# CompVis/stable-diffusion

Measured on AMD Instinct MI355X. Metric: 512x512 images/sec, SD-v1-4 50-step PLMS CFG=7.5, higher is better.
Workload: dtype f16

## Files before the change

include/sdmi.h:

```cpp
#ifndef SDMI_H_
#define SDMI_H_

#include <stdint.h>

#ifdef __cplusplus
extern "C" {
#endif

#define SDMI_ABI_VERSION 17

typedef struct sdmi_unet sdmi_unet;

typedef struct sdmi_unet_cfg {
  int32_t in_channels;
  int32_t out_channels;
  int32_t model_channels;
  int32_t num_res_blocks;
  int32_t n_levels;
  int32_t channel_mult[8];
  int32_t n_attention_resolutions;
  int32_t attention_resolutions[8];
  int32_t num_heads;
  int32_t transformer_depth;
  int32_t context_dim;
// ... 237 lines not shown
                      float* out, int64_t ldo, void* stream);

typedef struct sdmi_igemm_desc {
  const void* a0; const void* a1; const void* a2;
  int32_t c0, c1, c2, lda0, lda1, lda2;
  int32_t B, Hin, Win, Hout, Wout, ksize, stride, up;
  const void* w;
  int32_t N;
  int32_t mode;
  const float* bias; const float* rowvec; int32_t ld_rowvec;
  const float* residual; int32_t ldr;
  float* out_f32; void* out_f16; int32_t ldo;
  void* seg_dst[3]; int32_t seg_kind[3];
  int32_t heads, dh, ntok, ntok_pad, segC;
  int32_t splitk;
  float* splitk_ws; int64_t splitk_ws_floats;
  int32_t tile;
  int32_t dma;
  int32_t asym_pad;
  int32_t gn_n; void* gn_acc[2]; int32_t gn_cpg[2]; int32_t gn_cbase[2];
  int32_t* splitk_cnt; int32_t splitk_cnt_ints;
  int32_t split16;
  const float* f16_scale; float* lnp_out;
  const float* lnf_part; int32_t lnf_npart; float lnf_eps; const float* lnf_cs; const float* lnf_d;
  const float* pgn_gamma; const float* pgn_beta; float pgn_eps; int32_t pgn_silu;
  void* pgn_out; int32_t pgn_keep_f32; int32_t* pgn_applied;
  void* out_lo;
} sdmi_igemm_desc;
int sdmi_k_igemm(const sdmi_igemm_desc* d, void* stream);
int sdmi_k_igemm_tail(const sdmi_igemm_desc* d, const void* t0, const void* t1, const void* t2, int tail_c, int tail_ld, const void* tail_w,
                      int tail_kt, void* stream);
int sdmi_k_tail_split_range(int nkt, int nsplit, int split, int* begin, int* end);
int sdmi_k_igemm_up_phase(const sdmi_igemm_desc* d, void* stream);
int sdmi_k_up_phase_weights(const void* w_packed_f16, void* dst_f16, int N, int Cin, void* stream);
int sdmi_k_ff_tail(const sdmi_igemm_desc* proj_out, const void* ln_f16, const float* lnp, float ln_eps, const float* csd,
                   const void* wgg_f16, const void* wff2_f16, const float* bff2, const float* t, void* stream);
int sdmi_k_st_tail(const sdmi_igemm_desc* proj_out, const void* a_f16, const void* wo_f16, const float* bo, float* t, const float* ln_gamma,
                   float ln_eps, const float* csd, const void* wgg_f16, const void* wff2_f16, const float* bff2, void* stream);
int sdmi_k_gn_conv3(const sdmi_igemm_desc* conv, const float* x0, const float* x1, int c0, int c1, float* gn_ws, int64_t gn_ws_floats,
                    const float* gn_gamma, const float* gn_beta, float gn_eps, void* stream);
int sdmi_k_st_head(const float* x, float* gn_ws, int64_t gn_ws_floats, const float* gn_gamma, const float* gn_beta, float gn_eps,
                   const void* w_in3, const float* b_in, float* t, const float* ln_gamma, float ln_eps, const void* wqkv_f16,
                   const float* lnf_cs, const float* lnf_d, void* q, void* k, void* vt, int B, int ntok, int ntok_pad, int heads, int dh,
                   int C, void* stream);
int sdmi_k_st_mid(const void* a_f16, const void* wo_f16, const float* bo, float* t, const float* ln_gamma, float ln_eps, const void* wq_f16,
                  const float* lnf_cs, const float* lnf_d, void* q, int B, int ntok, int heads, int dh, int C, void* stream);
int sdmi_k_st_mid_ctx(const void* a_f16, const void* wo_f16, const float* bo, float* t, const float* ln_gamma, float ln_eps, const void* wq_f16,
                      const float* lnf_cs, const float* lnf_d, const void* ctx_k, const void* ctx_vt, int nkv, int nkv_pad, float scale, void* ao_out,
                      int B, int ntok, int heads, int dh, int C, void* stream);
int sdmi_k_ln_fold_prep(const void* w_f16, int N, int K, int ldw, const float* gamma, const float* beta, const float* bias,
                        float* cs, float* d, void* stream);
int sdmi_k_attention(const void* q, const void* k, const void* vt, void* out, int BH, int heads, int nq, int nkv,
                     int nkv_pad, int d, float scale, void* stream);
int sdmi_k_attention_split16(const void* q, const void* q_lo, const void* k, const void* k_lo, const void* vt, const void* vt_lo, void* out,
                             void* out_lo, int BH, int heads, int nq, int nkv, int nkv_pad, int d, float scale, void* stream);
int sdmi_k_attention_split16_causal(const void* q, const void* q_lo, const void* k, const void* k_lo, const void* vt, const void* vt_lo,
                                    void* out, void* out_lo, int BH, int heads, int n, int n_pad, int d, float scale, void* stream);
int sdmi_k_attention_causal(const void* q, const void* k, const void* vt, void* out, int BH, int heads, int n, int n_pad,
                            int d, float scale, void* stream);
int sdmi_k_groupnorm(const float* x0, const float* x1, int c0, int c1, int B, int HW, const float* gamma,
                     const float* beta, float eps, int silu, void* out_f16, float* out_f32, void* raw_f16, void* out_lo,
                     void* raw_lo, float* partial_ws, int64_t partial_floats, void* stream);
int64_t sdmi_k_groupnorm_ws_floats(int B, int HW);
int sdmi_k_groupnorm_film(const float* x0, const float* x1, int c0, int c1, int B, int HW, const float* gamma, const float* beta, float eps,
                          int silu, const float* film, int film_ld, void* out_f16, float* out_f32, void* raw_f16, void* out_lo, void* raw_lo,
                          float* partial_ws, int64_t partial_floats, void* stream);
int sdmi_k_layernorm(const float* x, const float* gamma, const float* beta, void* out_f16, int M, int C, float eps,
                     void* stream);
int sdmi_k_cast_f16(const float* x, void* out_f16, void* out_lo, int64_t n, void* stream);
int sdmi_k_split_heads(const float* src, int ld, int col0, void* dst, void* dst_lo, int kind, int B, int ntok, int ntok_pad, int heads, int dh,
                       void* stream);
int sdmi_k_geglu_split(const float* src, int M, int F, void* out, void* out_lo, void* stream);
int sdmi_k_layernorm_split(const float* x, const float* gamma, const float* beta, void* out, void* out_lo, int M, int C, float eps, void* stream);
int sdmi_k_timestep_embedding(const int64_t* t_i64, const float* t_f32, float* out, int B, int dim, void* stream);
int sdmi_k_small_linear(const float* in, int ld_in, const float* w, const float* bias, float* out, int ld_out, int B,
                        int N, int K, int silu_in, void* stream);
int sdmi_k_conv_in(const float* x_nchw, const float* w_oihw, const float* bias, float* out_nhwc, int B, int Cin, int H,
                   int W, int Cout, void* stream);
int sdmi_k_conv_out(const float* h_nhwc, const float* w_ohwi, const float* bias, float* out_nchw, int B, int H, int W,
                    int Cin, int Cout, void* stream);
int sdmi_k_conv_out32(const float* h_nhwc, const float* w_ohwi, const float* bias, float* out_nchw, int B, int H, int W,
                      int Cin, int Cout, void* stream);
int sdmi_k_conv_in64(const float* x_nchw, const float* w_oihw, const float* bias, float* out_nhwc, int B, int Cin, int H, int W,
                     int Cout, void* stream);
int sdmi_k_conv_out128(const float* h_nhwc, const float* w_ohwi, const float* bias, float* out_nchw, int B, int H, int W, int Cin,
                       int Cout, void* stream);
int sdmi_k_pack_conv_weight(const float* w_oihw, void* dst_f16, int O, int I, int KH, int KW, void* stream);
int sdmi_k_pack_conv_weight_src(const float* w_oihw, void* dst_f16, int O, int I, int KH, int KW, int c0, int c1, int c2, void* stream);
int sdmi_k_pack_conv_out(const float* w_oihw, float* dst_ohwi, int O, int I, void* stream);
int sdmi_k_pack_split3(const float* w, void* dst_f16, int N, int K, void* stream);
int sdmi_k_pack_conv_split3(const float* w_oihw, void* dst_f16, int O, int I, int KH, int KW, void* stream);
int sdmi_k_pointwise_nchw(const float* x, const float* w, const float* bias, float* out, int B, int Cin, int Cout, int HW,
                          float in_scale, void* stream);
int sdmi_k_pointwise_nchw128(const float* x, const float* w, const float* bias, float* out, int B, int Cin, int Cout, int HW,
                             float in_scale, void* stream);
int sdmi_k_softmax_rows(const float* S, void* P_f16, int rows, int cols, float scale, void* stream);
int sdmi_k_vq_quantize(const float* z, float z_scale, const float* codebook, float* norms_ws, int n_embed, int D, float* zq, int32_t* idx,
                       int B, int HW, void* stream);
int sdmi_k_resample2(const float* x, float* out_f32, void* out_f16, void* out_lo, int B, int H, int W, int C, int dir, void* stream);
int sdmi_k_patch_unfold(const float* x, const float* c, float* out, int B, int Cx, int Cc, int H, int W, int kh, int kw, int sy, int sx,
                        int l0, int nl, void* stream);
int sdmi_k_patch_fold(const float* o, const float* w, float* out, int B, int C, int H, int W, int kh, int kw, int sy, int sx, int uf, int df,
                      int norm_only, void* stream);
int sdmi_k_spatial_rescale(const float* x, const float* w, const float* bias, float* out, int B, int Cin, int H, int W, int n_stages,
                           int Cout, void* stream);
int sdmi_k_spatial_rescale_labels(const int32_t* labels, const float* w, const float* bias, float* out, int B, int Cin, int H, int W,
// ... 24 lines not shown
```

stable-diffusion_amd/_lib.py:

```python
import ctypes as C
import os

_HERE = os.path.dirname(os.path.abspath(__file__))
LIB_PATH = os.environ.get('SDMI_LIB_PATH') or os.path.join(_HERE, 'libsdmi.so')

c_f32p = C.c_void_p
c_ptr = C.c_void_p


class UNetCfg(C.Structure):
    _fields_ = [('in_channels', C.c_int32), ('out_channels', C.c_int32), ('model_channels', C.c_int32),
                ('num_res_blocks', C.c_int32), ('n_levels', C.c_int32), ('channel_mult', C.c_int32 * 8),
                ('n_attention_resolutions', C.c_int32), ('attention_resolutions', C.c_int32 * 8),
                ('num_heads', C.c_int32), ('transformer_depth', C.c_int32), ('context_dim', C.c_int32)]


class VaeCfg(C.Structure):
    _fields_ = [('ch', C.c_int32), ('out_ch', C.c_int32), ('n_levels', C.c_int32), ('ch_mult', C.c_int32 * 8),
                ('num_res_blocks', C.c_int32), ('in_channels', C.c_int32), ('z_channels', C.c_int32),
                ('embed_dim', C.c_int32)]


class UNetExt(C.Structure):
    _fields_ = [('attention_block', C.c_int32), ('resblock_updown', C.c_int32)]
# ... 152 lines not shown
    'sdmi_k_safety_head': (C.c_int, [c_ptr, c_ptr, c_ptr, c_ptr, c_ptr, c_ptr, c_ptr, c_ptr, C.c_int, C.c_int, C.c_int, C.c_int, c_ptr]),
    'sdmi_fe_ksize': (C.c_int, [C.c_int, C.c_int]),
    'sdmi_fe_coeffs': (C.c_int, [C.c_int, C.c_int, c_ptr, c_ptr]),
    'sdmi_fe_output_size': (C.c_int, [C.c_int, C.c_int, C.c_int, C.POINTER(C.c_int), C.POINTER(C.c_int)]),
    'sdmi_fe_workspace_bytes': (C.c_int64, [C.c_int] * 5),
    'sdmi_k_clip_feature_extract': (C.c_int, [c_ptr] + [C.c_int] * 7 + [c_ptr, c_ptr, C.c_int, c_ptr, c_ptr, C.c_int, C.POINTER(C.c_float),
                                              C.POINTER(C.c_float), c_ptr, C.c_int64, c_ptr, c_ptr, c_ptr]),
    'sdmi_knn_create': (C.c_int, [C.c_int, C.c_int64, C.POINTER(c_ptr)]),
    'sdmi_knn_destroy': (C.c_int, [c_ptr]),
    'sdmi_knn_set_rows': (C.c_int, [c_ptr, C.c_int64, C.c_int64, c_ptr, c_ptr]),
    'sdmi_knn_finalize': (C.c_int, [c_ptr, c_ptr]),
    'sdmi_knn_rows': (C.c_int64, [c_ptr]),
    'sdmi_knn_dim': (C.c_int, [c_ptr]),
    'sdmi_knn_workspace_bytes': (C.c_int64, [c_ptr, C.c_int, C.c_int]),
    'sdmi_knn_search': (C.c_int, [c_ptr, c_ptr, C.c_int, C.c_int, c_ptr, c_ptr, c_ptr, c_ptr, C.c_int64, c_ptr]),
    'sdmi_knn_condition': (C.c_int, [c_ptr, c_ptr, C.c_int, C.c_int, c_ptr, c_ptr, c_ptr, c_ptr, C.c_int64, c_ptr]),
    'sdmi_k_knn_inv_norm': (C.c_int, [c_ptr, C.c_int64, C.c_int, c_ptr, c_ptr]),
    'sdmi_k_knn_scan': (C.c_int, [c_ptr, c_ptr, C.c_int64, C.c_int, c_ptr, C.c_int, C.c_int, C.c_int64, c_ptr, c_ptr, c_ptr]),
    'sdmi_k_knn_merge': (C.c_int, [c_ptr, c_ptr, C.c_int, C.c_int, C.c_int, c_ptr, c_ptr, c_ptr]),
    'sdmi_k_knn_stream_read': (C.c_int, [c_ptr, C.c_int64, c_ptr, c_ptr]),
    'sdmi_k_knn_gather': (C.c_int, [c_ptr, c_ptr, C.c_int64, C.c_int, c_ptr, C.c_int, C.c_int, c_ptr, c_ptr, C.c_int64, c_ptr]),
    'sdmi_has_experiments': (C.c_int, []),
    'sdmi_k_igemm': (C.c_int, [C.POINTER(IGemmDesc), c_ptr]),
    'sdmi_k_igemm_tail': (C.c_int, [C.POINTER(IGemmDesc), c_ptr, c_ptr, c_ptr, C.c_int, C.c_int, c_ptr, C.c_int, c_ptr]),
    'sdmi_k_tail_split_range': (C.c_int, [C.c_int, C.c_int, C.c_int, C.POINTER(C.c_int), C.POINTER(C.c_int)]),
    'sdmi_k_igemm_up_phase': (C.c_int, [C.POINTER(IGemmDesc), c_ptr]),
    'sdmi_k_up_phase_weights': (C.c_int, [c_ptr, c_ptr, C.c_int, C.c_int, c_ptr]),
    'sdmi_tune_lookup': (C.c_int, [C.c_int] * 9 + [C.POINTER(C.c_int), C.POINTER(C.c_int)]),
    'sdmi_unet_skip_fold_plan': (C.c_int, [c_ptr, C.c_int, C.c_int, C.c_int, C.c_int, C.POINTER(C.c_int32), C.c_int]),
    'sdmi_k_ff_tail': (C.c_int, [C.POINTER(IGemmDesc), c_ptr, c_ptr, C.c_float, c_ptr, c_ptr, c_ptr, c_ptr, c_ptr, c_ptr]),
    'sdmi_k_gn_conv3': (C.c_int, [C.POINTER(IGemmDesc), c_ptr, c_ptr, C.c_int, C.c_int, c_ptr, C.c_int64, c_ptr, c_ptr, C.c_float, c_ptr]),
    'sdmi_k_st_mid_ctx': (C.c_int, [c_ptr, c_ptr, c_ptr, c_ptr, c_ptr, C.c_float, c_ptr, c_ptr, c_ptr, c_ptr, c_ptr, C.c_int, C.c_int, C.c_float, c_ptr,
                                    C.c_int, C.c_int, C.c_int, C.c_int, C.c_int, c_ptr]),
    'sdmi_k_st_tail': (C.c_int, [C.POINTER(IGemmDesc), c_ptr, c_ptr, c_ptr, c_ptr, c_ptr, C.c_float, c_ptr, c_ptr, c_ptr, c_ptr, c_ptr]),
    'sdmi_k_st_mid': (C.c_int, [c_ptr, c_ptr, c_ptr, c_ptr, c_ptr, C.c_float, c_ptr, c_ptr, c_ptr, c_ptr, C.c_int, C.c_int, C.c_int, C.c_int,
                                C.c_int, c_ptr]),
    'sdmi_k_st_head': (C.c_int, [c_ptr, c_ptr, C.c_int64, c_ptr, c_ptr, C.c_float, c_ptr, c_ptr, c_ptr, c_ptr, C.c_float, c_ptr, c_ptr, c_ptr,
                                 c_ptr, c_ptr, c_ptr, C.c_int, C.c_int, C.c_int, C.c_int, C.c_int, C.c_int, c_ptr]),
    'sdmi_k_attention_split16': (C.c_int, [c_ptr, c_ptr, c_ptr, c_ptr, c_ptr, c_ptr, c_ptr, c_ptr, C.c_int, C.c_int, C.c_int, C.c_int,
                                           C.c_int, C.c_int, C.c_float, c_ptr]),
    'sdmi_k_attention_split16_causal': (C.c_int, [c_ptr, c_ptr, c_ptr, c_ptr, c_ptr, c_ptr, c_ptr, c_ptr, C.c_int, C.c_int, C.c_int, C.c_int,
                                                  C.c_int, C.c_float, c_ptr]),
    'sdmi_k_attention_causal': (C.c_int, [c_ptr, c_ptr, c_ptr, c_ptr, C.c_int, C.c_int, C.c_int, C.c_int, C.c_int, C.c_float,
                                          c_ptr]),
    'sdmi_k_pointwise_nchw': (C.c_int, [c_ptr, c_ptr, c_ptr, c_ptr, C.c_int, C.c_int, C.c_int, C.c_int, C.c_float, c_ptr]),
    'sdmi_k_pointwise_nchw128': (C.c_int, [c_ptr, c_ptr, c_ptr, c_ptr, C.c_int, C.c_int, C.c_int, C.c_int, C.c_float, c_ptr]),
    'sdmi_k_softmax_rows': (C.c_int, [c_ptr, c_ptr, C.c_int, C.c_int, C.c_float, c_ptr]),
    'sdmi_k_gelu_erf': (C.c_int, [c_ptr, c_ptr, C.c_int64, c_ptr]),
    'sdmi_k_quick_gelu': (C.c_int, [c_ptr, c_ptr, C.c_int64, c_ptr]),
    'sdmi_k_quick_gelu_split': (C.c_int, [c_ptr, c_ptr, c_ptr, C.c_int64, c_ptr]),
    'sdmi_k_gelu_erf_split': (C.c_int, [c_ptr, c_ptr, c_ptr, C.c_int64, c_ptr]),
    'sdmi_k_attention': (C.c_int, [c_ptr, c_ptr, c_ptr, c_ptr, C.c_int, C.c_int, C.c_int, C.c_int, C.c_int, C.c_int,
                                   C.c_float, c_ptr]),
    'sdmi_k_groupnorm': (C.c_int, [c_ptr, c_ptr, C.c_int, C.c_int, C.c_int, C.c_int, c_ptr, c_ptr, C.c_float, C.c_int,
                                   c_ptr, c_ptr, c_ptr, c_ptr, c_ptr, c_ptr, C.c_int64, c_ptr]),
    'sdmi_k_groupnorm_ws_floats': (C.c_int64, [C.c_int, C.c_int]),
    'sdmi_k_groupnorm_film': (C.c_int, [c_ptr, c_ptr, C.c_int, C.c_int, C.c_int, C.c_int, c_ptr, c_ptr, C.c_float, C.c_int, c_ptr, C.c_int,
                                        c_ptr, c_ptr, c_ptr, c_ptr, c_ptr, c_ptr, C.c_int64, c_ptr]),
    'sdmi_k_layernorm': (C.c_int, [c_ptr, c_ptr, c_ptr, c_ptr, C.c_int, C.c_int, C.c_float, c_ptr]),
    'sdmi_k_cast_f16': (C.c_int, [c_ptr, c_ptr, c_ptr, C.c_int64, c_ptr]),
    'sdmi_k_split_heads': (C.c_int, [c_ptr, C.c_int, C.c_int, c_ptr, c_ptr, C.c_int, C.c_int, C.c_int, C.c_int, C.c_int, C.c_int,
                                     c_ptr]),
    'sdmi_k_geglu_split': (C.c_int, [c_ptr, C.c_int, C.c_int, c_ptr, c_ptr, c_ptr]),
    'sdmi_k_layernorm_split': (C.c_int, [c_ptr, c_ptr, c_ptr, c_ptr, c_ptr, C.c_int, C.c_int, C.c_float, c_ptr]),
    'sdmi_k_timestep_embedding': (C.c_int, [c_ptr, c_ptr, c_ptr, C.c_int, C.c_int, c_ptr]),
    'sdmi_k_small_linear': (C.c_int, [c_ptr, C.c_int, c_ptr, c_ptr, c_ptr, C.c_int, C.c_int, C.c_int, C.c_int,
                                      C.c_int, c_ptr]),
    'sdmi_k_conv_in': (C.c_int, [c_ptr, c_ptr, c_ptr, c_ptr, C.c_int, C.c_int, C.c_int, C.c_int, C.c_int, c_ptr]),
    'sdmi_k_conv_out': (C.c_int, [c_ptr, c_ptr, c_ptr, c_ptr, C.c_int, C.c_int, C.c_int, C.c_int, C.c_int, c_ptr]),
    'sdmi_k_pack_conv_weight': (C.c_int, [c_ptr, c_ptr, C.c_int, C.c_int, C.c_int, C.c_int, c_ptr]),
    'sdmi_k_pack_conv_weight_src': (C.c_int, [c_ptr, c_ptr, C.c_int, C.c_int, C.c_int, C.c_int, C.c_int, C.c_int, C.c_int, c_ptr]),
    'sdmi_k_conv_out32': (C.c_int, [c_ptr, c_ptr, c_ptr, c_ptr, C.c_int, C.c_int, C.c_int, C.c_int, C.c_int, c_ptr]),
    'sdmi_k_conv_in64': (C.c_int, [c_ptr, c_ptr, c_ptr, c_ptr, C.c_int, C.c_int, C.c_int, C.c_int, C.c_int, c_ptr]),
    'sdmi_k_conv_out128': (C.c_int, [c_ptr, c_ptr, c_ptr, c_ptr, C.c_int, C.c_int, C.c_int, C.c_int, C.c_int, c_ptr]),
    'sdmi_k_pack_conv_out': (C.c_int, [c_ptr, c_ptr, C.c_int, C.c_int, c_ptr]),
    'sdmi_k_pack_split3': (C.c_int, [c_ptr, c_ptr, C.c_int, C.c_int, c_ptr]),
    'sdmi_k_pack_conv_split3': (C.c_int, [c_ptr, c_ptr, C.c_int, C.c_int, C.c_int, C.c_int, c_ptr]),
    'sdmi_k_pack_geglu': (C.c_int, [c_ptr, c_ptr, c_ptr, c_ptr, C.c_int, C.c_int, c_ptr]),
    'sdmi_k_ln_fold_prep': (C.c_int, [c_ptr, C.c_int, C.c_int, C.c_int, c_ptr, c_ptr, c_ptr, c_ptr, c_ptr, c_ptr]),
    'sdmi_image_to_uint8': (C.c_int, [c_ptr, c_ptr, C.c_int, C.c_int, C.c_int, C.c_int, c_ptr]),
    'sdmi_range_check': (C.c_int, [C.c_int]),
    'sdmi_range_report': (C.c_int, [C.c_char_p, C.c_int]),
    'sdmi_tune_begin': (C.c_int, []),
    'sdmi_tune_round': (C.c_int, [C.c_int]),
    'sdmi_tune_end': (C.c_int, [C.c_char_p, C.POINTER(C.c_int)]),
    'sdmi_tune_dump': (C.c_int, [C.c_char_p, C.c_int]),
    'sdmi_profile_begin': (C.c_int, []),
    'sdmi_profile_end': (C.c_int, [C.c_char_p, C.c_int]),
    'sdmi_k_prefetch_lines': (C.c_int, [c_ptr, C.c_int64, c_ptr]),
    'sdmi_zero_page': (c_ptr, []),
}

_lib = None


class SdmiError(RuntimeError):
    pass


def load():
    global _lib
    if _lib is None:
        if not os.path.exists(LIB_PATH):
            raise SdmiError(f'{LIB_PATH} not found: build it with `python stable-diffusion_amd/build.py` '
                            '(the MI355X path has no fallback implementation)')
        lib = C.CDLL(LIB_PATH)
# ... 27 lines not shown
```

stable-diffusion_amd/build.py:

```python
import concurrent.futures as cf
import hashlib
import os
import subprocess
import sys

HERE = os.path.dirname(os.path.abspath(__file__))
CSRC = os.path.join(HERE, 'csrc')
EXTRA = os.environ.get('SDMI_CXXFLAGS', '').split()
LIB = os.path.join(HERE, os.environ.get('SDMI_LIB_OUT', 'libsdmi.so'))
OBJ = os.path.join(HERE, 'build' if os.path.basename(LIB) == 'libsdmi.so' else 'build_' + os.path.splitext(os.path.basename(LIB))[0])
SOURCES = ['igemm_t1.hip', 'igemm_t0.hip', 'igemm_t2.hip', 'igemm_h1.hip', 'igemm_h0.hip', 'igemm_h2.hip', 'igemm.hip', 'conv3halo.hip', 'gemm_split16.hip', 'rowchain.hip', 'gnconv.hip', 'range.hip', 'attn.hip', 'attn_wide.hip', 'attn_split16.hip', 'attn_wide_split16.hip', 'split_ops.hip', 'norm.hip', 'small.hip', 'sampler.hip', 'dpm.hip', 'inpaint.hip', 'patch.hip', 'vit.hip', 'knn.hip', 'textpool.hip', 'rescale.hip', 'feature_extractor.hip', 'fe_coeffs.cpp', 'weights.cpp', 'unet.cpp', 'vae.cpp', 'clip.cpp', 'bert.cpp', 'api.cpp', 'prof.cpp']
NO_CONTRACT = ('sampler.hip', 'dpm.hip', 'feature_extractor.hip', 'fe_coeffs.cpp')
FLAGS = ['--offload-arch=gfx950', '-O3', '-std=c++17', '-fPIC', '-munsafe-fp-atomics', '-Wall', '-Wno-unused-function',
         '-Wno-unused-variable']


def _hipcc():
    for c in (os.environ.get('HIPCC'), '/opt/rocm/bin/hipcc', 'hipcc'):
        if c and (not os.path.isabs(c) or os.path.exists(c)):
            return c
    raise RuntimeError('hipcc not found')


def _stamp():
    h = hashlib.sha256()
    for root in (CSRC, os.path.join(os.path.dirname(HERE), 'include')):
        for fn in sorted(os.listdir(root)):
            with open(os.path.join(root, fn), 'rb') as f:
                h.update(fn.encode())
                h.update(f.read())
    h.update(' '.join(FLAGS + EXTRA).encode())
    return h.hexdigest()


def is_current():
    stamp_file = os.path.join(OBJ, 'stamp')
    return os.path.exists(LIB) and os.path.exists(stamp_file) and open(stamp_file).read() == _stamp()


def build(force=False, verbose=True):
    os.makedirs(OBJ, exist_ok=True)
    stamp_file = os.path.join(OBJ, 'stamp')
    if not force and is_current():
        return LIB
    hipcc = _hipcc()
    stamp_now = _stamp()

    inc_dirs = (CSRC, os.path.join(os.path.dirname(HERE), 'include'))

    def deps_hash(src):
        import re
        seen, todo, h = set(), [os.path.join(CSRC, src)], hashlib.sha256()
        while todo:
            path = todo.pop()
            if path in seen:
                continue
            seen.add(path)
            with open(path, 'rb') as f:
                data = f.read()
            h.update(os.path.basename(path).encode())
            h.update(data)
            for inc in re.findall(rb'^\s*#\s*include\s*"([^"]+)"', data, re.M):
                for d in (os.path.dirname(path),) + inc_dirs:
                    cand = os.path.join(d, inc.decode())
# ... 37 lines not shown
```

stable-diffusion_amd/csrc/api.cpp:

```cpp
#include <string.h>

#include <new>

#include "prof.h"
#include "split16.h"
#include "unet.h"
#include "vae.h"
#include "clip.h"
#include "knn.h"
#include "rescale.h"
#include "fe_coeffs.h"
#include "feature_extractor.h"
#include "sampler_rows.h"

namespace sdmi {
static thread_local std::string g_err;
void set_error(const std::string& msg) { g_err = msg; }
int fail(const std::string& msg) { g_err = msg; return -1; }
}

struct sdmi_unet { sdmi::UNet impl; };
struct sdmi_vae { sdmi::Vae impl; };
struct sdmi_clip { sdmi::ClipText impl; };
struct sdmi_bert { sdmi::BertText impl; };
// ... 676 lines not shown
  if (launch_groupnorm(g, (hipStream_t)stream)) return -1;
  q.x0 = x0; q.x1 = x1; q.c0 = c0; q.c1 = c1; q.gn_acc = (const long long*)gn_ws; q.gn_gamma = gn_gamma; q.gn_beta = gn_beta; q.gn_eps = gn_eps;
  q.w = (const f16*)conv->w;
  return launch_gn_conv3(q, (hipStream_t)stream);
}
int sdmi_k_st_head(const float* x, float* gn_ws, int64_t gn_ws_floats, const float* gn_gamma, const float* gn_beta, float gn_eps,
                   const void* w_in3, const float* b_in, float* t, const float* ln_gamma, float ln_eps, const void* wqkv_f16,
                   const float* lnf_cs, const float* lnf_d, void* q, void* k, void* vt, int B, int ntok, int ntok_pad, int heads, int dh,
                   int C, void* stream) {
  SDMI_CHECK(x && gn_ws && gn_gamma && gn_beta, "st_head: null argument");
  SDMI_CHECK(gn_ws_floats >= gn_acc_words(B) * 2, "groupnorm workspace too small");
  SDMI_HIP_OK(hipMemsetAsync(gn_ws, 0, gn_acc_words(B) * sizeof(long long), (hipStream_t)stream));
  GroupNormParams g = GroupNormParams();
  g.x0 = x; g.c0 = C; g.B = B; g.HW = ntok; g.gamma = gn_gamma; g.beta = gn_beta; g.eps = gn_eps; g.stats_only = 1; g.acc = (long long*)gn_ws;
  if (launch_groupnorm(g, (hipStream_t)stream)) return -1;
  StHeadParams p = StHeadParams();
  p.x = x; p.gn_acc = (const long long*)gn_ws; p.gn_gamma = gn_gamma; p.gn_beta = gn_beta; p.gn_eps = gn_eps;
  p.w_in = (const f16*)w_in3; p.b_in = b_in; p.t = t; p.ln_gamma = ln_gamma; p.ln_eps = ln_eps; p.wqkv = (const f16*)wqkv_f16;
  p.lnf_cs = lnf_cs; p.lnf_d = lnf_d; p.q = (f16*)q; p.k = (f16*)k; p.vt = (f16*)vt;
  p.M = B * ntok; p.B = B; p.ntok = ntok; p.ntok_pad = ntok_pad; p.heads = heads; p.dh = dh; p.C = C;
  return launch_st_head(p, (hipStream_t)stream);
}
int sdmi_k_st_mid(const void* a_f16, const void* wo_f16, const float* bo, float* t, const float* ln_gamma, float ln_eps, const void* wq_f16,
                  const float* lnf_cs, const float* lnf_d, void* q, int B, int ntok, int heads, int dh, int C, void* stream) {
  StHeadParams p = StHeadParams();
  p.a16 = (const f16*)a_f16; p.w_in = (const f16*)wo_f16; p.b_in = bo; p.t = t; p.ln_gamma = ln_gamma; p.ln_eps = ln_eps;
  p.wqkv = (const f16*)wq_f16; p.lnf_cs = lnf_cs; p.lnf_d = lnf_d; p.q = (f16*)q;
  p.M = B * ntok; p.B = B; p.ntok = ntok; p.ntok_pad = ntok; p.heads = heads; p.dh = dh; p.C = C;
  return launch_st_mid(p, (hipStream_t)stream);
}
int sdmi_k_st_mid_ctx(const void* a_f16, const void* wo_f16, const float* bo, float* t, const float* ln_gamma, float ln_eps, const void* wq_f16,
                      const float* lnf_cs, const float* lnf_d, const void* ctx_k, const void* ctx_vt, int nkv, int nkv_pad, float scale, void* ao_out,
                      int B, int ntok, int heads, int dh, int C, void* stream) {
  StHeadParams p = StHeadParams();
  p.a16 = (const f16*)a_f16; p.w_in = (const f16*)wo_f16; p.b_in = bo; p.t = t; p.ln_gamma = ln_gamma; p.ln_eps = ln_eps;
  p.wqkv = (const f16*)wq_f16; p.lnf_cs = lnf_cs; p.lnf_d = lnf_d;
  p.ctx_k = (const f16*)ctx_k; p.ctx_vt = (const f16*)ctx_vt; p.ctx_nkv = nkv; p.ctx_nkv_pad = nkv_pad; p.ctx_scale = scale; p.ao_out = (f16*)ao_out;
  SDMI_CHECK(ctx_k && ctx_vt && ao_out, "st_mid_ctx: null argument");
  p.M = B * ntok; p.B = B; p.ntok = ntok; p.ntok_pad = ntok; p.heads = heads; p.dh = dh; p.C = C;
  return launch_st_mid(p, (hipStream_t)stream);
}
int sdmi_k_ln_fold_prep(const void* w_f16, int N, int K, int ldw, const float* gamma, const float* beta, const float* bias,
                        float* cs, float* d, void* stream) {
  return launch_ln_fold_prep((const f16*)w_f16, N, K, ldw, gamma, beta, bias, cs, d, (hipStream_t)stream);
}
int sdmi_k_attention(const void* q, const void* k, const void* vt, void* out, int BH, int heads, int nq, int nkv,
                     int nkv_pad, int d, float scale, void* stream) {
  AttnParams a = AttnParams();
  a.q = (const f16*)q; a.k = (const f16*)k; a.vt = (const f16*)vt; a.out = (f16*)out;
  a.BH = BH; a.heads = heads; a.nq = nq; a.nkv = nkv; a.nkv_pad = nkv_pad; a.d = d; a.scale = scale;
  if (const char* e = getenv("SDMI_ATTN_NW")) a.nw = atoi(e);
  return launch_attention(a, (hipStream_t)stream);
}
int sdmi_k_attention_split16(const void* q, const void* q_lo, const void* k, const void* k_lo, const void* vt, const void* vt_lo, void* out,
                             void* out_lo, int BH, int heads, int nq, int nkv, int nkv_pad, int d, float scale, void* stream) {
  AttnSplitParams a = AttnSplitParams();
  a.q = (const f16*)q; a.q_lo = (const f16*)q_lo; a.k = (const f16*)k; a.k_lo = (const f16*)k_lo; a.vt = (const f16*)vt;
  a.vt_lo = (const f16*)vt_lo; a.out = (f16*)out; a.out_lo = (f16*)out_lo;
  a.BH = BH; a.heads = heads; a.nq = nq; a.nkv = nkv; a.nkv_pad = nkv_pad; a.d = d; a.scale = scale;
  return launch_attention_split16(a, (hipStream_t)stream);
}
int64_t sdmi_k_groupnorm_ws_floats(int B, int HW) { (void)HW; return gn_acc_words(B) * 2; }
int sdmi_k_groupnorm(const float* x0, const float* x1, int c0, int c1, int B, int HW, const float* gamma,
                     const float* beta, float eps, int silu, void* out_f16, float* out_f32, void* raw_f16, void* out_lo,
                     void* raw_lo, float* partial_ws, int64_t partial_floats, void* stream) {
  SDMI_CHECK(partial_floats >= gn_acc_words(B) * 2, "groupnorm workspace too small");
  SDMI_HIP_OK(hipMemsetAsync(partial_ws, 0, gn_acc_words(B) * sizeof(long long), (hipStream_t)stream));
  GroupNormParams g = GroupNormParams();
  g.x0 = x0; g.x1 = x1; g.c0 = c0; g.c1 = c1; g.B = B; g.HW = HW; g.gamma = gamma; g.beta = beta; g.eps = eps;
  g.silu = silu; g.out_f16 = (f16*)out_f16; g.out_f32 = out_f32; g.raw_f16 = (f16*)raw_f16; g.out_lo = (f16*)out_lo; g.raw_lo = (f16*)raw_lo;
  g.acc = (long long*)partial_ws;
  return launch_groupnorm(g, (hipStream_t)stream);
}
int sdmi_k_groupnorm_film(const float* x0, const float* x1, int c0, int c1, int B, int HW, const float* gamma, const float* beta, float eps,
                          int silu, const float* film, int film_ld, void* out_f16, float* out_f32, void* raw_f16, void* out_lo, void* raw_lo,
                          float* partial_ws, int64_t partial_floats, void* stream) {
  SDMI_CHECK(partial_floats >= gn_acc_words(B) * 2, "groupnorm workspace too small");
  SDMI_HIP_OK(hipMemsetAsync(partial_ws, 0, gn_acc_words(B) * sizeof(long long), (hipStream_t)stream));
  GroupNormParams g = GroupNormParams();
  g.x0 = x0; g.x1 = x1; g.c0 = c0; g.c1 = c1; g.B = B; g.HW = HW; g.gamma = gamma; g.beta = beta; g.eps = eps;
  g.silu = silu; g.out_f16 = (f16*)out_f16; g.out_f32 = out_f32; g.raw_f16 = (f16*)raw_f16; g.out_lo = (f16*)out_lo; g.raw_lo = (f16*)raw_lo;
  g.film = film; g.film_ld = film_ld;
  g.acc = (long long*)partial_ws;
  return launch_groupnorm(g, (hipStream_t)stream);
}
int sdmi_k_layernorm(const float* x, const float* gamma, const float* beta, void* out_f16, int M, int C, float eps,
                     void* stream) {
  return launch_layernorm(x, gamma, beta, (f16*)out_f16, M, C, eps, (hipStream_t)stream);
}
int sdmi_k_cast_f16(const float* x, void* out_f16, void* out_lo, int64_t n, void* stream) {
  return launch_cast_f16(x, (f16*)out_f16, (f16*)out_lo, n, (hipStream_t)stream);
}
int sdmi_k_split_heads(const float* src, int ld, int col0, void* dst, void* dst_lo, int kind, int B, int ntok, int ntok_pad, int heads, int dh,
                       void* stream) {
  return launch_split_heads(src, ld, col0, (f16*)dst, (f16*)dst_lo, kind, B, ntok, ntok_pad, heads, dh, (hipStream_t)stream);
}
int sdmi_k_geglu_split(const float* src, int M, int F, void* out, void* out_lo, void* stream) {
  return launch_geglu_split(src, M, F, (f16*)out, (f16*)out_lo, (hipStream_t)stream);
}
int sdmi_k_layernorm_split(const float* x, const float* gamma, const float* beta, void* out, void* out_lo, int M, int C, float eps, void* stream) {
  return launch_layernorm_split(x, gamma, beta, (f16*)out, (f16*)out_lo, M, C, eps, (hipStream_t)stream);
}
int sdmi_k_timestep_embedding(const int64_t* t_i64, const float* t_f32, float* out, int B, int dim, void* stream) {
  return launch_timestep_embedding(t_i64, t_f32, out, B, dim, (hipStream_t)stream);
}
int sdmi_k_small_linear(const float* in, int ld_in, const float* w, const float* bias, float* out, int ld_out, int B,
// ... 88 lines not shown
```

stable-diffusion_amd/csrc/attn.hip:

```cpp
#include <type_traits>

#include "common.h"
#include "prof.h"

namespace sdmi {
namespace {

constexpr int KVT = 64;
typedef float f32x2 __attribute__((ext_vector_type(2)));
typedef _Float16 f16x2 __attribute__((ext_vector_type(2)));
typedef unsigned u32x4 __attribute__((ext_vector_type(4)));

template <int N>
__device__ __forceinline__ void wait_dma() {
  static_assert(N >= 0 && N <= 44, "add the literal");
  switch (N) {
#define SDMI_VM(k) case k: asm volatile("s_waitcnt vmcnt(" #k ")" ::: "memory"); break
    SDMI_VM(0); SDMI_VM(1); SDMI_VM(2); SDMI_VM(3); SDMI_VM(4); SDMI_VM(5); SDMI_VM(6); SDMI_VM(7); SDMI_VM(8); SDMI_VM(9);
    SDMI_VM(10); SDMI_VM(11); SDMI_VM(12); SDMI_VM(13); SDMI_VM(14); SDMI_VM(15); SDMI_VM(16); SDMI_VM(17); SDMI_VM(18);
    SDMI_VM(19); SDMI_VM(20); SDMI_VM(21); SDMI_VM(22); SDMI_VM(23); SDMI_VM(24); SDMI_VM(25); SDMI_VM(26); SDMI_VM(27);
    SDMI_VM(28); SDMI_VM(29); SDMI_VM(30); SDMI_VM(31); SDMI_VM(32); SDMI_VM(33); SDMI_VM(34); SDMI_VM(35); SDMI_VM(36);
    SDMI_VM(37); SDMI_VM(38); SDMI_VM(39); SDMI_VM(40); SDMI_VM(41); SDMI_VM(42); SDMI_VM(43); SDMI_VM(44);
#undef SDMI_VM
  }
// ... 446 lines not shown
    const float m1 = xch[(DVT * 16) * 64], l1 = xch[(DVT * 16 + 1) * 64];
    const float m = fmaxf(m_run, m1);
    const float a0 = __builtin_amdgcn_exp2f(m_run - m), a1 = __builtin_amdgcn_exp2f(m1 - m);
#pragma unroll
    for (int dt = 0; dt < DVT; ++dt)
#pragma unroll
      for (int r = 0; r < 16; ++r) o[dt][r] = a0 * o[dt][r] + a1 * xch[(dt * 16 + r) * 64];
    l_run = a0 * l_run + a1 * l1;
  }

  float l_tot;
  if (ONES) {
    constexpr int rl = D % 32, r_l = (rl & 3) + 4 * (rl >> 3), lg_l = (rl >> 2) & 1;
    float a = o[D / 32][r_l], b = a;
    swap_halves(a, b);
    l_tot = lg_l == 0 ? a : b;
  } else {
    l_tot = sum_across_halves(l_run);
  }
  const float inv = 1.0f / l_tot;
  const int q = q0 + l31;
  if (q < p.nq) {
    const int b = bh / p.heads, head = bh - b * p.heads;
    f16* orow = p.out + ((size_t)b * p.nq + q) * ((size_t)p.heads * D) + (size_t)head * D;
#pragma unroll
    for (int dt = 0; dt < DVT; ++dt)
#pragma unroll
      for (int r4 = 0; r4 < 4; ++r4) {
        const int dd = dt * 32 + 8 * r4 + 4 * lg;
        if (dd < D) {
          f16x4 v = {(f16)(o[dt][r4 * 4 + 0] * inv), (f16)(o[dt][r4 * 4 + 1] * inv), (f16)(o[dt][r4 * 4 + 2] * inv),
                     (f16)(o[dt][r4 * 4 + 3] * inv)};
          SDMI_ST(f16x4, orow + dd, v);
        }
      }
  }
#endif
}

#ifndef SDMI_ATTN_KVS_DEFAULT
#define SDMI_ATTN_KVS_DEFAULT 1
#endif
template <int D>
int launch_d(const AttnParams& p, hipStream_t stream) {
  int nw = p.nw;
  if (nw <= 0) {
    const int slices = cdiv(p.nq, 32);
    nw = (slices >= 8 && p.nq > 1024) ? 8 : (slices >= 4 ? 4 : 2);
  }
  dim3 grid(cdiv(p.nq, 32 * nw), p.BH);
  static const std::string pname_long = std::string("attn_d") + std::to_string(D) + "_self";
  static const std::string pname_short = std::string("attn_d") + std::to_string(D) + "_ctx";
  ProfScope ps((p.nkv >= 256 ? pname_long : pname_short).c_str(), 4.0 * p.BH * (double)p.nq * p.nkv * D, 2.0 * p.BH * D * (2.0 * p.nq + 2.0 * p.nkv), stream);
  constexpr int DNS = (D > 128) ? 3 : 4;
  const int kvs_env = getenv("SDMI_ATTN_KVS") ? atoi(getenv("SDMI_ATTN_KVS")) : SDMI_ATTN_KVS_DEFAULT;
  const bool kvs2 = D == 40 && nw == 8 && !p.causal && p.nkv % (2 * KVT) == 0 && p.nkv >= 32 * KVT && kvs_env != 0 && (p.nkv <= 64 * KVT || kvs_env == 2);
  if (!p.causal && (p.nkv * D) % 8 == 0) {
#ifdef SDMI_ABLATE
    static const int abl = getenv("SDMI_ATTN_ABL") ? atoi(getenv("SDMI_ATTN_ABL")) : 0;
#else
    constexpr int abl = 0;
#endif
    if (D == 40 && nw == 8 && abl) {
#ifdef SDMI_ABLATE
      if constexpr (D == 40) {
        switch (abl) {
          case 1: SDMI_LAUNCH((attn_dma_kernel<D, 8, DNS, false, 1>), grid, dim3(512), 0, stream, p); break;
          case 2: SDMI_LAUNCH((attn_dma_kernel<D, 8, DNS, false, 2>), grid, dim3(512), 0, stream, p); break;
          case 3: SDMI_LAUNCH((attn_dma_kernel<D, 8, DNS, false, 3>), grid, dim3(512), 0, stream, p); break;
          case 4: SDMI_LAUNCH((attn_dma_kernel<D, 8, DNS, false, 4>), grid, dim3(512), 0, stream, p); break;
          case 5: SDMI_LAUNCH((attn_dma_kernel<D, 8, DNS, false, 5>), grid, dim3(512), 0, stream, p); break;
          default: SDMI_LAUNCH((attn_dma_kernel<D, 8, DNS, false, 6>), grid, dim3(512), 0, stream, p); break;
        }
      }
#endif
    } else if (nw == 8 && kvs2) {
      if constexpr (D == 40) SDMI_LAUNCH((attn_dma_kernel<D, 16, DNS, false, 0, 2>), grid, dim3(1024), 0, stream, p);
    } else if (nw == 8) SDMI_LAUNCH((attn_dma_kernel<D, 8, DNS, false>), grid, dim3(512), 0, stream, p);
    else if (nw == 4) SDMI_LAUNCH((attn_dma_kernel<D, 4, DNS, false>), grid, dim3(256), 0, stream, p);
    else SDMI_LAUNCH((attn_dma_kernel<D, 2, DNS, false>), grid, dim3(128), 0, stream, p);
  } else if (p.causal) {
    if constexpr (D == 32 || D == 64 || D == 128) SDMI_LAUNCH((attn_kernel<D, 2, true>), dim3(cdiv(p.nq, 64), p.BH), dim3(128), 0, stream, p);
    else return fail("causal attention is instantiated for head dims 32 / 64 / 128");
  } else if (nw == 8) SDMI_LAUNCH((attn_kernel<D, 8, false>), grid, dim3(512), 0, stream, p);
  else if (nw == 4) SDMI_LAUNCH((attn_kernel<D, 4, false>), grid, dim3(256), 0, stream, p);
  else SDMI_LAUNCH((attn_kernel<D, 2, false>), grid, dim3(128), 0, stream, p);
  SDMI_HIP_OK(hipGetLastError());
  return 0;
}

}

static int launch_attention_impl(const AttnParams& p, hipStream_t stream);
int launch_attention(const AttnParams& p, hipStream_t stream) {
  const int rc = launch_attention_impl(p, stream);
  if (rc == 0 && range_check_enabled()) return range_scan("attention output", p.out, (int64_t)p.BH * p.nq * p.d, stream);
  return rc;
}
static int launch_attention_impl(const AttnParams& p, hipStream_t stream) {
  SDMI_CHECK(p.BH > 0 && p.nq > 0 && p.nkv > 0 && p.heads > 0 && p.BH % p.heads == 0, "bad attention shape");
  SDMI_CHECK(p.nkv_pad % 8 == 0 && p.nkv_pad >= p.nkv, "nkv_pad must be a multiple of 8 and >= nkv");
  SDMI_CHECK(!p.causal || p.nq == p.nkv, "causal attention needs nq == nkv");
  switch (p.d) {
    case 24: return launch_d<24>(p, stream);
    case 32: return launch_d<32>(p, stream);
    case 40: return launch_d<40>(p, stream);
    case 48: return launch_d<48>(p, stream);
    case 64: return launch_d<64>(p, stream);
    case 80: return launch_d<80>(p, stream);
    case 96: return launch_d<96>(p, stream);
    case 128: return launch_d<128>(p, stream);
    case 160: return launch_d<160>(p, stream);
    default: return launch_attention_wide(p, stream);
  }
}

}
```

stable-diffusion_amd/csrc/common.h:

```cpp
#pragma once
#include <hip/hip_runtime.h>
#include <stdint.h>
#include <algorithm>
#include <string>

#include "tape.h"

typedef _Float16 f16;
typedef _Float16 f16x2 __attribute__((ext_vector_type(2)));
typedef _Float16 f16x4 __attribute__((ext_vector_type(4)));
typedef _Float16 f16x8 __attribute__((ext_vector_type(8)));
typedef float f32x4 __attribute__((ext_vector_type(4)));
typedef float f32x16 __attribute__((ext_vector_type(16)));

#ifdef __HIPCC__
__device__ __forceinline__ float gn_apply_elem(float v, float mean, float rstd, float gamma, float beta, int silu) {
  float t = __builtin_fmaf((v - mean) * rstd, gamma, beta);
  if (silu) t = t * __builtin_amdgcn_rcpf(1.0f + __expf(-t));
  return t;
}
__device__ __forceinline__ float gn_apply_film_elem(float v, float mean, float rstd, float gamma, float beta, float scale, float shift,
                                                    int silu) {
  float t = __builtin_fmaf((v - mean) * rstd, gamma, beta);
  t = __builtin_fmaf(t, 1.0f + scale, shift);
// ... 208 lines not shown
int launch_ff_tail(const FfTailParams& p, hipStream_t stream);

struct StHeadParams {
  const f16* a16 = nullptr;
  const float* x = nullptr;
  const long long* gn_acc = nullptr;
  const float* gn_gamma = nullptr; const float* gn_beta = nullptr; float gn_eps = 1e-6f;
  const f16* w_in = nullptr;
  const float* b_in = nullptr;
  float* t = nullptr;
  const float* ln_gamma = nullptr;
  float ln_eps = 1e-5f;
  const f16* wqkv = nullptr;
  const float* lnf_cs = nullptr; const float* lnf_d = nullptr;
  f16* q = nullptr; f16* k = nullptr;
  f16* vt = nullptr;
  int M = 0, B = 0, ntok = 0, ntok_pad = 0, heads = 0, dh = 0, C = 0;
  const f16* ctx_k = nullptr; const f16* ctx_vt = nullptr; int ctx_nkv = 0, ctx_nkv_pad = 0; float ctx_scale = 0.f; f16* ao_out = nullptr;
#ifdef SDMI_RC_TIMING
  long long* dbg = nullptr;
#endif
};
bool st_head_supported(int C, int M, int ntok, int ntok_pad, int heads, int dh);
int launch_st_head(const StHeadParams& p, hipStream_t stream);
int launch_st_mid(const StHeadParams& p, hipStream_t stream);

struct GnConvParams {
  const float* x0 = nullptr; const float* x1 = nullptr; int c0 = 0, c1 = 0;
  const long long* gn_acc = nullptr;
  const float* gn_gamma = nullptr; const float* gn_beta = nullptr; float gn_eps = 1e-5f;
  const f16* w = nullptr;
#ifdef SDMI_RC_TIMING
  long long* dbg = nullptr;
#endif
  IGemmParams epi;
};
bool gn_conv3_supported(int B, int H, int W, int c0, int c1, int Cout);
int launch_gn_conv3(const GnConvParams& p, hipStream_t stream);

struct AttnParams {
  const f16* q = nullptr;
  const f16* k = nullptr;
  const f16* vt = nullptr;
  f16* out = nullptr;
  int BH = 0, heads = 0, nq = 0, nkv = 0, nkv_pad = 0, d = 0;
  float scale = 1.f;
  int nw = 0;
  int causal = 0;
  int prio = 0;
  int pingpong = 0;
};
int launch_attention(const AttnParams& p, hipStream_t stream);
int launch_attention_wide(const AttnParams& p, hipStream_t stream);

struct GroupNormParams {
  const float* x0 = nullptr; const float* x1 = nullptr; int c0 = 0, c1 = 0;
  int B = 0, HW = 0;
  const float* gamma = nullptr; const float* beta = nullptr; float eps = 1e-5f;
  int silu = 0;
  int stats_only = 0;
  int skip_stats = 0;
  f16* out_f16 = nullptr;
  float* out_f32 = nullptr;
  f16* raw_f16 = nullptr;
  f16* out_lo = nullptr;
  f16* raw_lo = nullptr;
  const float* film = nullptr; int film_ld = 0;
  long long* acc = nullptr;
};
constexpr int GN_SLOTS = 8;
constexpr int GN_MAX_CALLS = 96;
constexpr int GN_WORDS = 4;
constexpr int GN_STRIDE = 16;
static inline int64_t gn_acc_words(int B) { return (int64_t)B * 32 * GN_SLOTS * GN_STRIDE; }
int launch_groupnorm(const GroupNormParams& p, hipStream_t stream);

int launch_layernorm(const float* x, const float* gamma, const float* beta, f16* out, int M, int C, float eps,
                     hipStream_t stream, float* out_f32 = nullptr);
int launch_cast_f16(const float* x, f16* out, f16* out_lo, int64_t n, hipStream_t stream);

int launch_timestep_embedding(const int64_t* t_i64, const float* t_f32, float* out, int B, int dim, hipStream_t s);
int launch_small_linear(const float* in, int ld_in, const float* w, const float* bias, float* out, int ld_out,
                        int B, int N, int K, int silu_in, hipStream_t s);
int launch_ctx1_broadcast(const f16* vt, int ld_v, f16* ao, int B, int ntok, int C, hipStream_t s);
int launch_conv_in(const float* x_nchw, const float* w, const float* bias, float* out_nhwc, int B, int Cin, int H,
                   int W, int Cout, hipStream_t s, int gn_n = 0, long long* const* gn_acc = nullptr, const int* gn_cpg = nullptr,
                   const int* gn_cbase = nullptr);
int launch_conv_out(const float* h_nhwc, const float* w_khwc, const float* bias, float* out_nchw, int B, int H, int W,
                    int Cin, int Cout, hipStream_t s);

struct DpmStepParams {
  const float* eps_model = nullptr;
  int cfg = 0; float scale = 1.f;
  const float* x = nullptr;
  const float* m_prev = nullptr;
  float alpha_s = 1.f, sigma_s = 0.f;
  float cx = 1.f, a = 0.f, inv_r0 = 0.f;
  int order = 1;
  float* m_out = nullptr;
  float* x_next = nullptr;
  int64_t n = 0;
};
int launch_dpm_step(const DpmStepParams& p, hipStream_t s);

struct DpmModelValueParams {
  const float* eps_model = nullptr;
// ... 103 lines not shown
```

Before: 3.904.

## Add register-resident single-pass attention kernel for short-sequence d80/d160 heads

Adds a new attention kernel for head dims 80 and 160 with at most 256 keys. Each wave holds all keys in registers, computes the full score row with MFMA, runs one softmax without online rescaling, and prefetches K and V across steps. A rule table sends the 16x16 self- and cross-attention and the 32x32 cross-attention to this kernel by default, with environment overrides. It aims to cut the online-softmax and tiling overhead of the general kernel on small shapes, at the cost of more register pressure and extra template instantiations.

```diff
diff --git a/include/sdmi.h b/include/sdmi.h
--- a/include/sdmi.h
+++ b/include/sdmi.h
@@ -313,6 +313,7 @@
                         float* cs, float* d, void* stream);
 int sdmi_k_attention(const void* q, const void* k, const void* vt, void* out, int BH, int heads, int nq, int nkv,
                      int nkv_pad, int d, float scale, void* stream);
+int sdmi_attn_small_takes(int d, int nq, int nkv, int causal, int knob);
 int sdmi_k_attention_split16(const void* q, const void* q_lo, const void* k, const void* k_lo, const void* vt, const void* vt_lo, void* out,
                              void* out_lo, int BH, int heads, int nq, int nkv, int nkv_pad, int d, float scale, void* stream);
 int sdmi_k_attention_split16_causal(const void* q, const void* q_lo, const void* k, const void* k_lo, const void* vt, const void* vt_lo,
diff --git a/stable-diffusion_amd/_lib.py b/stable-diffusion_amd/_lib.py
--- a/stable-diffusion_amd/_lib.py
+++ b/stable-diffusion_amd/_lib.py
@@ -228,6 +228,7 @@
     'sdmi_k_gelu_erf_split': (C.c_int, [c_ptr, c_ptr, c_ptr, C.c_int64, c_ptr]),
     'sdmi_k_attention': (C.c_int, [c_ptr, c_ptr, c_ptr, c_ptr, C.c_int, C.c_int, C.c_int, C.c_int, C.c_int, C.c_int,
                                    C.c_float, c_ptr]),
+    'sdmi_attn_small_takes': (C.c_int, [C.c_int, C.c_int, C.c_int, C.c_int, C.c_int]),
     'sdmi_k_groupnorm': (C.c_int, [c_ptr, c_ptr, C.c_int, C.c_int, C.c_int, C.c_int, c_ptr, c_ptr, C.c_float, C.c_int,
                                    c_ptr, c_ptr, c_ptr, c_ptr, c_ptr, c_ptr, C.c_int64, c_ptr]),
     'sdmi_k_groupnorm_ws_floats': (C.c_int64, [C.c_int, C.c_int]),
diff --git a/stable-diffusion_amd/build.py b/stable-diffusion_amd/build.py
--- a/stable-diffusion_amd/build.py
+++ b/stable-diffusion_amd/build.py
@@ -9,7 +9,7 @@
 EXTRA = os.environ.get('SDMI_CXXFLAGS', '').split()
 LIB = os.path.join(HERE, os.environ.get('SDMI_LIB_OUT', 'libsdmi.so'))
 OBJ = os.path.join(HERE, 'build' if os.path.basename(LIB) == 'libsdmi.so' else 'build_' + os.path.splitext(os.path.basename(LIB))[0])
-SOURCES = ['igemm_t1.hip', 'igemm_t0.hip', 'igemm_t2.hip', 'igemm_h1.hip', 'igemm_h0.hip', 'igemm_h2.hip', 'igemm.hip', 'conv3halo.hip', 'gemm_split16.hip', 'rowchain.hip', 'gnconv.hip', 'range.hip', 'attn.hip', 'attn_wide.hip', 'attn_split16.hip', 'attn_wide_split16.hip', 'split_ops.hip', 'norm.hip', 'small.hip', 'sampler.hip', 'dpm.hip', 'inpaint.hip', 'patch.hip', 'vit.hip', 'knn.hip', 'textpool.hip', 'rescale.hip', 'feature_extractor.hip', 'fe_coeffs.cpp', 'weights.cpp', 'unet.cpp', 'vae.cpp', 'clip.cpp', 'bert.cpp', 'api.cpp', 'prof.cpp']
+SOURCES = ['igemm_t1.hip', 'igemm_t0.hip', 'igemm_t2.hip', 'igemm_h1.hip', 'igemm_h0.hip', 'igemm_h2.hip', 'igemm.hip', 'conv3halo.hip', 'gemm_split16.hip', 'rowchain.hip', 'gnconv.hip', 'range.hip', 'attn.hip', 'attn_small.hip', 'attn_wide.hip', 'attn_split16.hip', 'attn_wide_split16.hip', 'split_ops.hip', 'norm.hip', 'small.hip', 'sampler.hip', 'dpm.hip', 'inpaint.hip', 'patch.hip', 'vit.hip', 'knn.hip', 'textpool.hip', 'rescale.hip', 'feature_extractor.hip', 'fe_coeffs.cpp', 'weights.cpp', 'unet.cpp', 'vae.cpp', 'clip.cpp', 'bert.cpp', 'api.cpp', 'prof.cpp']
 NO_CONTRACT = ('sampler.hip', 'dpm.hip', 'feature_extractor.hip', 'fe_coeffs.cpp')
 FLAGS = ['--offload-arch=gfx950', '-O3', '-std=c++17', '-fPIC', '-munsafe-fp-atomics', '-Wall', '-Wno-unused-function',
          '-Wno-unused-variable']
diff --git a/stable-diffusion_amd/csrc/api.cpp b/stable-diffusion_amd/csrc/api.cpp
--- a/stable-diffusion_amd/csrc/api.cpp
+++ b/stable-diffusion_amd/csrc/api.cpp
@@ -752,6 +752,7 @@
   if (const char* e = getenv("SDMI_ATTN_NW")) a.nw = atoi(e);
   return launch_attention(a, (hipStream_t)stream);
 }
+int sdmi_attn_small_takes(int d, int nq, int nkv, int causal, int knob) { return attn_small_takes(d, nq, nkv, causal, knob); }
 int sdmi_k_attention_split16(const void* q, const void* q_lo, const void* k, const void* k_lo, const void* vt, const void* vt_lo, void* out,
                              void* out_lo, int BH, int heads, int nq, int nkv, int nkv_pad, int d, float scale, void* stream) {
   AttnSplitParams a = AttnSplitParams();
diff --git a/stable-diffusion_amd/csrc/attn.hip b/stable-diffusion_amd/csrc/attn.hip
--- a/stable-diffusion_amd/csrc/attn.hip
+++ b/stable-diffusion_amd/csrc/attn.hip
@@ -522,6 +522,14 @@
   static const std::string pname_long = std::string("attn_d") + std::to_string(D) + "_self";
   static const std::string pname_short = std::string("attn_d") + std::to_string(D) + "_ctx";
   ProfScope ps((p.nkv >= 256 ? pname_long : pname_short).c_str(), 4.0 * p.BH * (double)p.nq * p.nkv * D, 2.0 * p.BH * D * (2.0 * p.nq + 2.0 * p.nkv), stream);
+  if constexpr (D == 80 || D == 160) {
+    const int small_env = getenv("SDMI_ATTN_SMALL") ? atoi(getenv("SDMI_ATTN_SMALL")) : 1;
+    int snw = (p.nw <= 0 || small_env == 2) ? attn_small_takes(D, p.nq, p.nkv, p.causal, small_env) : 0;
+    if (snw) {
+      if (const char* e = getenv("SDMI_ATTN_SMALL_NW")) snw = atoi(e);
+      return launch_attention_small(p, snw, stream);
+    }
+  }
   constexpr int DNS = (D > 128) ? 3 : 4;
   const int kvs_env = getenv("SDMI_ATTN_KVS") ? atoi(getenv("SDMI_ATTN_KVS")) : SDMI_ATTN_KVS_DEFAULT;
   const bool kvs2 = D == 40 && nw == 8 && !p.causal && p.nkv % (2 * KVT) == 0 && p.nkv >= 32 * KVT && kvs_env != 0 && (p.nkv <= 64 * KVT || kvs_env == 2);
@@ -561,6 +569,21 @@
 
 }
 
+namespace {
+struct AttnSmallRule { int d, nq_lo, nq_hi, nkv_lo, nkv_hi, nw; };
+const AttnSmallRule kAttnSmallRules[] = {
+    {160,    1,  256,   1,  256,  1},
+    { 80,    1,  256,   1,  256,  1},
+    { 80,  257, 1024,   1,  128,  2},
+};
+}
+int attn_small_takes(int d, int nq, int nkv, int causal, int knob) {
+  if (knob == 0 || !attn_small_supported(d, nq, nkv, causal)) return 0;
+  for (const AttnSmallRule& r : kAttnSmallRules)
+    if (d == r.d && nq >= r.nq_lo && nq <= r.nq_hi && nkv >= r.nkv_lo && nkv <= r.nkv_hi) return r.nw;
+  return knob == 2 ? (nq > 256 ? 2 : 1) : 0;
+}
+
 static int launch_attention_impl(const AttnParams& p, hipStream_t stream);
 int launch_attention(const AttnParams& p, hipStream_t stream) {
   const int rc = launch_attention_impl(p, stream);
diff --git a/stable-diffusion_amd/csrc/attn_small.hip b/stable-diffusion_amd/csrc/attn_small.hip
--- /dev/null
+++ b/stable-diffusion_amd/csrc/attn_small.hip
@@ -0,0 +1,158 @@
+#include "common.h"
+
+namespace sdmi {
+namespace {
+
+template <int D, int NKB>
+__global__ void __launch_bounds__(256) attn_small_kernel(const AttnParams p) {
+#if defined(__HIP_DEVICE_COMPILE__)
+  static_assert(D % 16 == 0 && NKB >= 1 && NKB <= 8, "whole k-steps over the head dim; at most 256 keys");
+  constexpr int DKS = D / 16;
+  constexpr int DVT = (D + 31) / 32;
+  constexpr int NST = NKB * 2;
+  constexpr int KPF = D > 80 ? 3 : 4;
+  constexpr int VPF = D > 80 ? 6 : 8;
+
+  const int lane = threadIdx.x & 63;
+  const int wave = __builtin_amdgcn_readfirstlane(threadIdx.x >> 6);
+  const int l31 = lane & 31, lg = lane >> 5;
+  const int bh = blockIdx.y;
+  const int q0 = (blockIdx.x * (blockDim.x >> 6) + wave) * 32;
+  if (q0 >= p.nq) return;
+  const f16* Qg = p.q + (size_t)bh * p.nq * D;
+  const f16* Kg = p.k + (size_t)bh * p.nkv * D;
+  const f16* Vg = p.vt + (size_t)bh * D * p.nkv_pad;
+
+  f16x8 qf[DKS];
+  {
+    const f16* qp = Qg + min(q0 + l31, p.nq - 1) * D + lg * 8;
+#pragma unroll
+    for (int ks = 0; ks < DKS; ++ks) qf[ks] = *(const f16x8*)(qp + ks * 16);
+  }
+  const int prow = (l31 & ~12) | ((l31 & 4) << 1) | ((l31 & 8) >> 1);
+  f16x8 kf[NKB][DKS];
+  auto load_k = [&](int kb) {
+    const int key = kb == NKB - 1 ? min(kb * 32 + prow, p.nkv - 1) : kb * 32 + prow;
+    const f16* kp = Kg + key * D + lg * 8;
+#pragma unroll
+    for (int ks = 0; ks < DKS; ++ks) kf[kb][ks] = *(const f16x8*)(kp + ks * 16);
+  };
+  f16x8 vf[NST][DVT];
+  auto load_v = [&](int st) {
+    int col = st * 16 + lg * 8;
+    if (st >= NST - 2) col = min(col, p.nkv_pad - 8);
+#pragma unroll
+    for (int dt = 0; dt < DVT; ++dt) {
+      const int row = dt * 32 + 31 < D ? dt * 32 + l31 : min(dt * 32 + l31, D - 1);
+      vf[st][dt] = *(const f16x8*)(Vg + row * p.nkv_pad + col);
+    }
+  };
+
+  constexpr int KPFE = KPF < NKB ? KPF : NKB, VPFE = VPF < NST ? VPF : NST, VPER = (VPFE + KPFE - 1) / KPFE;
+  const f32x16 zero16 = {0.f, 0.f, 0.f, 0.f, 0.f, 0.f, 0.f, 0.f, 0.f, 0.f, 0.f, 0.f, 0.f, 0.f, 0.f, 0.f};
+  f32x16 s[NKB];
+#pragma unroll
+  for (int kb = 0; kb < KPFE; ++kb) load_k(kb);
+#pragma unroll
+  for (int kb = 0; kb < NKB; ++kb) {
+    if (kb + KPFE < NKB) {
+      load_k(kb + KPFE);
+    } else {
+#pragma unroll
+      for (int st = (kb + KPFE - NKB) * VPER; st < (kb + KPFE - NKB + 1) * VPER && st < VPFE; ++st) load_v(st);
+    }
+    __builtin_amdgcn_sched_barrier(0);
+#pragma unroll
+    for (int ks = 0; ks < DKS; ++ks)
+      s[kb] = __builtin_amdgcn_mfma_f32_32x32x16_f16(kf[kb][ks], qf[ks], ks == 0 ? zero16 : s[kb], 0, 0, 0);
+  }
+
+#pragma unroll
+  for (int r = 0; r < 16; ++r) {
+    const int kv = (NKB - 1) * 32 + (r & 3) + 4 * ((r >> 2) & 1) + 8 * lg + 16 * (r >> 3);
+    if (kv >= p.nkv) s[NKB - 1][r] = -1e30f;
+  }
+  float mx = -1e30f;
+#pragma unroll
+  for (int kb = 0; kb < NKB; ++kb)
+#pragma unroll
+    for (int r = 0; r < 16; ++r) mx = fmaxf(mx, s[kb][r]);
+  mx = fmaxf(mx, __shfl_xor(mx, 32));
+  const float sc = p.scale * 1.4426950408889634f;
+  const float m = mx * sc;
+  f16x8 pf[NST];
+  float l4[4] = {0.f, 0.f, 0.f, 0.f};
+  auto exp_step = [&](int st) {
+#pragma unroll
+    for (int e = 0; e < 8; ++e) {
+      const f16 h = (f16)__builtin_amdgcn_exp2f(fmaf(s[st >> 1][8 * (st & 1) + e], sc, -m));
+      pf[st][e] = h;
+      l4[e & 3] += (float)h;
+    }
+  };
+  exp_step(0);
+
+  f32x16 o[DVT];
+#pragma unroll
+  for (int st = 0; st < NST; ++st) {
+    if (st + VPFE < NST) load_v(st + VPFE);
+    __builtin_amdgcn_sched_barrier(0);
+    if (st + 1 < NST) exp_step(st + 1);
+#pragma unroll
+    for (int dt = 0; dt < DVT; ++dt)
+      o[dt] = __builtin_amdgcn_mfma_f32_32x32x16_f16(vf[st][dt], pf[st], st == 0 ? zero16 : o[dt], 0, 0, 0);
+  }
+  float l = (l4[0] + l4[1]) + (l4[2] + l4[3]);
+  l += __shfl_xor(l, 32);
+
+  const float inv = 1.0f / l;
+  const int q = q0 + l31;
+  if (q < p.nq) {
+    const int b = bh / p.heads, head = bh - b * p.heads;
+    f16* orow = p.out + ((size_t)b * p.nq + q) * ((size_t)p.heads * D) + (size_t)head * D;
+#pragma unroll
+    for (int dt = 0; dt < DVT; ++dt)
+#pragma unroll
+      for (int r4 = 0; r4 < 4; ++r4) {
+        const int dd = dt * 32 + 8 * r4 + 4 * lg;
+        if (dd < D) {
+          f16x4 v = {(f16)(o[dt][r4 * 4 + 0] * inv), (f16)(o[dt][r4 * 4 + 1] * inv), (f16)(o[dt][r4 * 4 + 2] * inv),
+                     (f16)(o[dt][r4 * 4 + 3] * inv)};
+          SDMI_ST(f16x4, orow + dd, v);
+        }
+      }
+  }
+#endif
+}
+
+template <int D>
+int launch_small_d(const AttnParams& p, int nw, hipStream_t stream) {
+  const dim3 grid(cdiv(cdiv(p.nq, 32), nw), p.BH), block(64 * nw);
+  switch (cdiv(p.nkv, 32)) {
+    case 1: SDMI_LAUNCH((attn_small_kernel<D, 1>), grid, block, 0, stream, p); break;
+    case 2: SDMI_LAUNCH((attn_small_kernel<D, 2>), grid, block, 0, stream, p); break;
+    case 3: SDMI_LAUNCH((attn_small_kernel<D, 3>), grid, block, 0, stream, p); break;
+    case 4: SDMI_LAUNCH((attn_small_kernel<D, 4>), grid, block, 0, stream, p); break;
+    case 5: SDMI_LAUNCH((attn_small_kernel<D, 5>), grid, block, 0, stream, p); break;
+    case 6: SDMI_LAUNCH((attn_small_kernel<D, 6>), grid, block, 0, stream, p); break;
+    case 7: SDMI_LAUNCH((attn_small_kernel<D, 7>), grid, block, 0, stream, p); break;
+    default: SDMI_LAUNCH((attn_small_kernel<D, 8>), grid, block, 0, stream, p); break;
+  }
+  SDMI_HIP_OK(hipGetLastError());
+  return 0;
+}
+
+}
+
+bool attn_small_supported(int d, int nq, int nkv, int causal) {
+  return (d == 80 || d == 160) && !causal && nq > 0 && nkv > 0 && nkv <= 256;
+}
+
+int launch_attention_small(const AttnParams& p, int nw, hipStream_t stream) {
+  SDMI_CHECK(attn_small_supported(p.d, p.nq, p.nkv, p.causal), "attn_small_kernel: d = 80 / 160, non-causal, at most 256 keys");
+  SDMI_CHECK(nw == 1 || nw == 2 || nw == 4, "attn_small_kernel: 1, 2 or 4 waves per workgroup");
+  SDMI_CHECK((int64_t)p.nq * p.d < (1ll << 31) && (int64_t)p.d * p.nkv_pad < (1ll << 31), "attn_small_kernel: 32-bit offsets inside a head");
+  return p.d == 80 ? launch_small_d<80>(p, nw, stream) : launch_small_d<160>(p, nw, stream);
+}
+
+}
diff --git a/stable-diffusion_amd/csrc/common.h b/stable-diffusion_amd/csrc/common.h
--- a/stable-diffusion_amd/csrc/common.h
+++ b/stable-diffusion_amd/csrc/common.h
@@ -284,6 +284,9 @@
 };
 int launch_attention(const AttnParams& p, hipStream_t stream);
 int launch_attention_wide(const AttnParams& p, hipStream_t stream);
+bool attn_small_supported(int d, int nq, int nkv, int causal);
+int launch_attention_small(const AttnParams& p, int nw, hipStream_t stream);
+int attn_small_takes(int d, int nq, int nkv, int causal, int knob);
 
 struct GroupNormParams {
   const float* x0 = nullptr; const float* x1 = nullptr; int c0 = 0, c1 = 0;
```

Result: faster. 3.956, median of 6 (+1.3%).
